# hdm0922/PathTracerDemo

Hardware: AMD Instinct MI355X
Metric: Msamples/sec at 1920x1080, 1 spp ReSTIR DI; per-pixel L2 vs WebGPU ref (higher is better)
Workload: dtype f32; 1 GPU; c3_interior_32 reuse 1920x1080, 1 spp/frame (configs[2]); frame=1920x1080, band_rows_per_gpu=1080, parallelism=row-bands x1

## Files before the change

pathtracerdemo_amd/csrc/ptx_api.cpp:

```cpp
#include <hip/hip_runtime.h>

#include <algorithm>
#include <cmath>
#include <cstdarg>
#include <cstdlib>
#include <cstdio>
#include <cstring>
#include <new>
#include <string>
#include <unordered_map>
#include <vector>

#include "ptx_internal.h"

namespace ptx {


[[maybe_unused]] static const char *const kShippedKnobs[] = {"COMM_TIMEOUT_S", "DEBUG_FILL", "HALO_PROXY_US"};
#if defined(PTX_WG_TIMES)
static const char *const kBuildKind = "wgt";
#elif defined(PTX_AB_BUILD)
static const char *const kBuildKind = "ab";
#else
static const char *const kBuildKind = "product";
// ... 351 lines not shown
    if (mats.size() != 8u * subs.size()) return fail(h, PTX_E_SCENE, "material / sub-mesh tables disagree");
    for (size_t k = 0; k < subs.size(); ++k) std::memcpy(&subs[k].pad, &mats[8u * k + 5u], 4);
    if (int rc = upload(h, h->d_tris, tris.data(), tris.size() * sizeof(float))) return rc;
    if (int rc = upload(h, h->d_nodes, nodes.data(), nodes.size() * sizeof(NodePair))) return rc;
    if (int rc = upload(h, h->d_subs, subs.data(), subs.size() * sizeof(SubRoot))) return rc;
    h->n_subs = (uint32_t)subs.size();
    if (int rc = upload(h, h->d_insts, insts.data(), std::max<size_t>(1, insts.size()) * sizeof(Inst))) return rc;
    if (int rc = upload(h, h->d_mats, mats.data(), mats.size() * sizeof(float))) return rc;
    if (int rc = upload(h, h->d_tverts, tverts.data(), tverts.size() * sizeof(float))) return rc;
    h->n_tris = (uint32_t)(tris.size() / 12);
    h->n_nodes = (uint32_t)nodes.size();
    h->n_inst = n_inst;
    h->max_depth = max_depth;
    h->stack_depth = max_depth + 2u;
    if ((size_t)h->stack_depth * kBlock * 4u > 160u * 1024u)
        return fail(h, PTX_E_SCENE, "BLAS depth %u needs more LDS than a CU has", max_depth);
    h->layout_valid = true;
    for (auto &c : h->ctx) c.surf_valid = false;
    gbuf_key_drop_all(h);
    return PTX_OK;
}

Scene make_scene(ptx_handle *h) {
    Scene sc{};
    std::memcpy(sc.U, h->uniform, sizeof sc.U);
    sc.S = (const uint32_t *)h->d_scene.p;
    sc.G = (const uint32_t *)h->d_geometry.p;
    sc.tris = (const float4 *)h->d_tris.p;
    sc.nodes = (const NodePair *)h->d_nodes.p;
    sc.subs = (const SubRoot *)h->d_subs.p;
    sc.insts = (const Inst *)h->d_insts.p;
    sc.mats = (const float4 *)h->d_mats.p;
    sc.tverts = (const float4 *)h->d_tverts.p;
    sc.n_inst = h->n_inst;
    sc.n_subs = h->n_subs;
    sc.width = h->cfg.width;
    sc.height = h->cfg.height;
    sc.row_begin = h->cfg.row_begin;
    sc.row_end = h->cfg.row_end;
    sc.counters = (h->cfg.flags & PTX_FLAG_COUNT_WORK) ? (unsigned long long *)h->d_counters.p : nullptr;
    sc.census = (h->cfg.flags & PTX_FLAG_ROW_CENSUS) ? (unsigned long long *)h->d_census.p : nullptr;
    sc.frame_color = (float4 *)h->d_frame_color.p;
#ifdef PTX_WG_TIMES
    sc.wgt = (unsigned long long *)h->d_wgt.p;
#endif
    return sc;
}

void resolve_event(TimedLaunch &t, ptx_handle *h) {
    if (!t.pending) return;
    float ms = 0.0f;
    if (hipEventSynchronize(t.stop) == hipSuccess && hipEventElapsedTime(&ms, t.start, t.stop) == hipSuccess) {
        h->ms_total[t.pass] += ms;
        h->launches[t.pass] += 1;
    }
    t.pending = false;
}

static uint32_t seg_pixels(const ptx_handle *h) {
    static const uint32_t env_px = (uint32_t)ab_knob("SEG_PX", 0);
    if (env_px >= 256u && env_px <= 8192u && env_px % 256u == 0u) return env_px;
    const size_t npx = (size_t)h->band_h * h->cfg.width;
    if ((h->cfg.pipeline == PTX_PIPELINE_RESTIR && restir_pipe()) || (h->cfg.pipeline == PTX_PIPELINE_MCPT && mcpt_pipe()) ||
        h->cfg.pipeline == PTX_PIPELINE_RESTIR_GI) {
        const size_t p = (npx / 1152u + 128u) / 256u * 256u;
        return (uint32_t)std::min<size_t>(4096u, std::max<size_t>(kWaveSegPixels, p));
// ... 1763 lines not shown
```

pathtracerdemo_amd/csrc/ptx_device.h:

```cpp
#pragma once

#include <hip/hip_runtime.h>
#include <stdint.h>

namespace ptx {

constexpr uint32_t STRIDE_INSTANCE = 33u;
constexpr uint32_t STRIDE_LIGHT = 18u;
constexpr uint32_t STRIDE_DESCRIPTOR = 6u;
constexpr uint32_t STRIDE_MATERIAL = 15u;
constexpr uint32_t STRIDE_VERTEX = 8u;
constexpr float RECONNECTION_DISTANCE = 0.1f;
constexpr float RECONNECTION_ROUGHNESS = 0.5f;
constexpr float INF_F = 1e11f;
constexpr float EPS_F = 1e-4f;
constexpr float PI_F = 3.141592f;
constexpr float ENV_C = 0.5f;
constexpr uint32_t LIGHT_DIRECTION = 0u, LIGHT_POINT = 1u, LIGHT_RECT = 2u, LIGHT_ENV = 3u;
constexpr uint32_t LOBE_LAMBERT = 0u, LOBE_GGX = 1u, LOBE_LIGHT = 3u;

enum : uint32_t {
    U_W = 0, U_H = 1, U_VPINV = 4, U_CAMPOS = 20, U_FRAME = 23, U_OFF_DESC = 24, U_OFF_MAT = 25,
    U_OFF_LIGHT = 26, U_OFF_CDF = 27, U_OFF_INDEX = 28, U_OFF_SUBROOT = 29, U_OFF_BLAS = 30,
    U_INST_COUNT = 31, U_LIGHT_COUNT = 32
};

constexpr uint32_t LEAF_BIT = 0x80000000u;
constexpr uint32_t LEAF_FIRST_MASK = 0x00FFFFFFu;

struct alignas(16) NodePair {
    float x[4], y[4], z[4];
    uint32_t lref, rref, pad0, pad1;
};
struct alignas(16) SubRoot {
    float x[2], y[2], z[2];
    uint32_t ref;
    uint32_t pad;
};
struct alignas(16) Inst {
    float m[16];
    float minv[16];
    uint32_t mesh, sub_base, nsub, tri_base;
    float wlo[3], wpad;
    float whi[3], wscale;
};
constexpr uint32_t kInstIdentity = 0x80000000u;

struct Scene {
    uint32_t U[33];
    const uint32_t *S;
    const uint32_t *G;
    const float4 *tris;
    const NodePair *nodes;
    const SubRoot *subs;
    const Inst *insts;
    const float4 *mats;
    const float4 *tverts;
    uint32_t n_inst, n_subs;
    uint32_t width, height, row_begin, row_end;
    unsigned long long *counters;
    unsigned long long *census;
    float4 *frame_color;
#ifdef PTX_WG_TIMES
    unsigned long long *wgt;
#endif
};

enum : uint32_t { KID_TRACE = 1, KID_GBUF, KID_INIT_START, KID_INIT_STEP, KID_FINAL_START, KID_FINAL_STEP,
                  KID_TEMP_START, KID_TEMP_COMBINE, KID_SPAT_START, KID_JOB_STEP, KID_SPAT_COMBINE };
#ifdef PTX_WG_TIMES
struct WaveTimer {
    unsigned long long *buf;
    unsigned long long t0;
    uint32_t kid;
    __device__ WaveTimer(unsigned long long *b, uint32_t k) : buf(b), t0(__builtin_amdgcn_s_memrealtime()), kid(k) {}
    __device__ ~WaveTimer() {
        if (!buf || __lane_id() != 0u) return;
        const unsigned long long t1 = __builtin_amdgcn_s_memrealtime();
        const unsigned long long i = atomicAdd(buf, 1ull);
        if (i >= (1ull << 20)) return;
        unsigned long long *r = buf + 4u + 4u * i;
        r[0] = t0;
        r[1] = t1;
        r[2] = ((unsigned long long)kid << 32) | blockIdx.x;
        r[3] = ((unsigned long long)(threadIdx.x >> 6) << 32) | (unsigned long long)__builtin_amdgcn_s_getreg((31 << 11) | 4);
    }
};
#define PTX_WAVE_TIMER(sc, k) WaveTimer wave_timer_((sc).wgt, (k))
constexpr uint32_t KID_BATCH = 12;
constexpr uint32_t KID_BATCH_DBG = 15;
// ... 725 lines not shown
    if ((COUNT || PROF) && counted) {
        atomicAdd(&sc.counters[CNT_RAYS], 1ull);
        atomicAdd(&sc.counters[CNT_INST], (unsigned long long)sc.n_inst);
        atomicAdd(&sc.counters[CNT_AABB], (unsigned long long)n_aabb);
        atomicAdd(&sc.counters[CNT_TRI], (unsigned long long)n_tri);
        if (best.valid) atomicAdd(&sc.counters[CNT_HITS], 1ull);
    }
    if (best.valid) {
        best.t = vy;
        if (!ANY && want_pos) complete_hit(sc, ray, eps, best, insts);
    }
    return best;
}

constexpr uint32_t kLdsTableMax = 24576u;
__host__ __device__ __forceinline__ uint32_t tables_lds_bytes(const Scene &sc) {
    return ((sc.n_subs * (uint32_t)sizeof(SubRoot) + 15u) & ~15u) + sc.n_inst * (uint32_t)sizeof(Inst);
}
__host__ __device__ __forceinline__ bool tables_fit_lds(const Scene &sc) { return tables_lds_bytes(sc) <= kLdsTableMax; }
struct LdsTables { const SubRoot *subs; const Inst *insts; };
__device__ __forceinline__ LdsTables stage_tables(const Scene &sc, uint32_t *lds) {
    SubRoot *l_subs = reinterpret_cast<SubRoot *>(lds);
    Inst *l_insts = reinterpret_cast<Inst *>(lds + ((sc.n_subs * (uint32_t)sizeof(SubRoot) + 15u) & ~15u) / 4u);
    const uint32_t *gs = reinterpret_cast<const uint32_t *>(sc.subs);
    uint32_t *ls = reinterpret_cast<uint32_t *>(l_subs);
    for (uint32_t i = threadIdx.x; i < sc.n_subs * (uint32_t)(sizeof(SubRoot) / 4u); i += blockDim.x) ls[i] = gs[i];
    const uint32_t *gi = reinterpret_cast<const uint32_t *>(sc.insts);
    uint32_t *li = reinterpret_cast<uint32_t *>(l_insts);
    for (uint32_t i = threadIdx.x; i < sc.n_inst * (uint32_t)(sizeof(Inst) / 4u); i += blockDim.x) li[i] = gi[i];
    __syncthreads();
    return LdsTables{l_subs, l_insts};
}

template <bool COUNT, bool PROF = false>
__device__ __forceinline__ Hit trace_core(const Scene &sc, Ray ray, PassEps eps, uint32_t *stack, uint32_t stride,
                                          float t_max = 1e10f) {
    return trace_core_tab<COUNT, PROF>(sc, sc.subs, sc.insts, ray, eps, stack, stride, t_max);
}
template <bool COUNT>
__device__ __attribute__((noinline)) Hit trace_ray(const Scene &sc, Ray ray, PassEps eps, uint32_t *stack,
                                                  uint32_t stride) {
    return trace_core<COUNT>(sc, ray, eps, stack, stride);
}

}
```

pathtracerdemo_amd/csrc/ptx_launch.h:

```cpp
#pragma once

#include <hip/hip_runtime.h>

#include "ptx_device.h"

namespace ptx {

constexpr int kTile = 16;
constexpr int kBlock = 256;

int env_knob(const char *key, int dflt);
#ifdef PTX_AB_BUILD
inline int ab_knob(const char *key, int dflt) { return env_knob(key, dflt); }
#else
constexpr int ab_knob(const char *, int dflt) { return dflt; }
#endif

inline size_t stack_lds_bytes(uint32_t depth) { return (size_t)depth * kBlock * sizeof(uint32_t); }

hipError_t launch_gbuffer(const Scene &sc, uint4 *gbuf, uint32_t stack_depth, hipStream_t s);
hipError_t launch_init(const Scene &sc, const uint4 *gbuf, uint4 *reservoir, uint32_t stack_depth, hipStream_t s);
hipError_t launch_final(const Scene &sc, const uint4 *gbuf, const uint4 *reservoir, float4 *accum,
                        uint32_t stack_depth, hipStream_t s);
hipError_t launch_mcpt(const Scene &sc, float4 *accum, uint32_t stack_depth, hipStream_t s);
hipError_t launch_present(const float4 *tex, uint32_t W, uint32_t H, uint32_t cw, uint32_t ch, bool bgra,
                          uint32_t *out, hipStream_t s);

struct DnWin {
    uint32_t y0;
    uint32_t rows;
    uint32_t c0, c1;
};
struct DnImage {
    const float4 *own, *halo;
    uint32_t o0, o1;
};
hipError_t launch_denoise_guide(const Scene &sc, const uint4 *gbuf, float4 *guide, float sigma_plane, hipStream_t s);
hipError_t launch_denoise_guide_halo(const Scene &sc, const uint4 *texels, uint32_t top, uint32_t bottom, float4 *guide,
                                     float sigma_plane, hipStream_t s);
hipError_t launch_denoise_variance(uint32_t W, const DnWin &win, const DnImage &img, const float4 *guide, float4 *out,
                                   hipStream_t s);
hipError_t launch_denoise_atrous(uint32_t W, const DnWin &win, uint32_t step, const float4 *in, const float4 *guide,
                                 float4 *out, float sigma_lum, bool last, hipStream_t s);
hipError_t launch_denoise_temporal(uint32_t W, uint32_t H, const DnWin &win, const float *vp_prev, float alpha_min,
                                   uint32_t mode, uint32_t prev_y0, uint32_t prev_rows, const float4 *guide,
                                   const float4 *frame, const float4 *accum, const float4 *pguide, const float4 *phist,
                                   const float2 *pmom, float4 *hist, float2 *mom, unsigned long long *clip, hipStream_t s);
hipError_t launch_denoise_variance_moments(uint32_t W, const DnWin &win, const float4 *hist, const float2 *mom,
                                           const float4 *guide, float4 *out, hipStream_t s);
// ... 119 lines not shown
```

pathtracerdemo_amd/csrc/ptx_reuse.hip:

```cpp
#include "ptx_wave_common.h"

namespace ptx {

constexpr uint32_t SALT_TEMPORAL = 0x54454D50u, SALT_SPATIAL = 0x53504154u;

enum : uint32_t { JS_HDR, JS_F, JS_CUR, JS_NRM, JS_PREV, JS_RRF, JS_COUNT };
constexpr uint32_t kJobFresh = 1u << 24;
constexpr uint32_t kResReuseLayout = 0x100u;
#ifndef PTX_JOB_FRESH
#define PTX_JOB_FRESH 1
#endif

struct Job {
    uint32_t i, length, phase, seed1, idx, matref;
    uint32_t k, lab;
    bool shift, rok;
    int32_t ref;
    int32_t dom;
    f3 f;
    float prod;
    Surface cur;
    f3 prev;
    float beta, rr_p;
    f3 rr_f;
// ... 198 lines not shown
                const f3 Ld = normalize(r);
                gl = fabsf(dot(get_light(sc, (uint32_t)XL.id).dir, Ld)) / dot(r, r);
            }
            s.prod = hyb ? s.prod / s.beta : s.prod / (gl * s.beta);
            Le = l_emit<true>(XL, s.cur);
            s.phase = 1u;
            const float dist = length(XL.pos - s.cur.pos);
            o = s.cur.pos; d = (XL.pos - s.cur.pos) / dist; remain = dist;
            vis = true;
            ray = go = ok;
        }
        if (!go) A.jres[jid] = make_float4(0.0f, 0.0f, 0.0f, 0.0f);
    }
    const uint32_t idx = g.rbase + wave_alloc(g.l_ray, ray ? 1u : 0u);
    if (ray) {
        s.idx = idx;
        put_ray(g.rays, idx, o, d, remain, vis ? Q_VIS : Q_CLOSEST);
        if (vis) g.res_out[2u * idx] = make_float4(0.0f, Le.x, Le.y, Le.z);
    }
    return go;
}

__device__ __forceinline__ void job_finish(const Seg &g, const JobLists &JL, const ReuseArgs &A, bool live,
                                           const Job &s, uint32_t jid) {
    if (live) job_store(A, jid, s);
    const bool fold = live && A.fold_last && s.phase == 1u;
    if (fold) A.jres[jid] = make_float4(asf(s.idx), asf(g.out_sel), 0.0f, asf(kJobPending));
    job_keep(g, JL, live && !fold, live && s.phase == 1u, jid);
}

#ifndef JOB_STEP_WAVES
#define JOB_STEP_WAVES 4
#endif
__device__ __forceinline__ uint32_t job_step_segment(const Scene &sc, const WaveBufs &w, uint32_t round,
                                                     const ReuseArgs &A, uint32_t *lds) {
    const JobLists JL = job_lists(w, lds);
    const Seg g = seg_begin(w, round, lds);
    uint32_t nh;
    const uint32_t n = split_count(g, nh);
    for (uint32_t base = 0; base < n; base += WB) {
        const uint32_t q = base + threadIdx.x;
        bool emit = false;
        uint32_t jid = 0u;
        Job s;
        if (q < n) {
            jid = split_at(g, JL, q, nh);
            job_load(sc, A, jid, s);
            if (s.phase != 1u) {
                bool ok = true;
                Surface next;
                uint32_t nref = 0u;
                if (s.phase == 0u) {
                    const Hit h = get_hit(g.res_in, s.idx);
                    ok = h.valid;
                    if (ok) {
                        next = surface_at(sc, h.s, h.pos);
                        nref = mat_index(sc, h.s.inst, h.s.mat);
                    }
                } else {
                    const uint4 *rv = res_of(A, s.ref);
                    const Compact cc = gdecode(s.phase == 2u ? rv[4] : rc_next(rv, rv[5].x));
                    next = get_surface(sc, cc);
                    nref = mat_index(sc, cc.inst, cc.mat);
                    if (s.phase == 2u) {
                        const Hit h = get_hit(g.res_in, s.idx);
                        ok = !(h.valid && h.t < length(next.pos - s.cur.pos) * 0.999f);
                    }
                }
                if (!ok) {
                    A.jres[jid] = make_float4(0.0f, 0.0f, 0.0f, 0.0f);
                } else {
                    const f3 V = normalize(s.prev - s.cur.pos);
                    const f3 L = normalize(next.pos - s.cur.pos);
                    s.f = s.f * (bsdf(s.cur, L, V) * fabsf(dot(s.cur.nrm, L)));
                    if (s.phase == 2u || (!s.shift && job_hyb(s) && s.i + 1u == s.k))
                        s.prod = s.prod * rc_geo(s.cur.pos, next);
                    s.prev = s.cur.pos;
                    s.cur = next;
                    s.matref = nref;
                    s.i += 1u;
                    emit = true;
                }
            } else {
                const float4 a = g.res_in[2u * s.idx];
                s.f = s.f * (mk(a.y, a.z, a.w) * a.x);
                const float qv = s.prod;
                const bool valid = qv > 0.0f && qv <= 3.402823466e38f;
                A.jres[jid] = valid ? make_float4(s.f.x, s.f.y, s.f.z, qv) : make_float4(0.0f, 0.0f, 0.0f, 0.0f);
            }
        }
        const bool live = job_emit(sc, g, A, emit, s, jid, 0u);
        job_finish(g, JL, A, live, s, jid);
    }
    job_seg_end(w, g, JL);
    return *g.l_ray;
}
__global__ __launch_bounds__(WB) __attribute__((amdgpu_waves_per_eu(JOB_STEP_WAVES, 8)))
void wjob_step(Scene sc, WaveBufs w, uint32_t round, ReuseArgs A) {
    PTX_WAVE_TIMER(sc, KID_JOB_STEP | (w.seg_base ? 0x80u : 0u));
    __shared__ uint32_t lds[3];
    (void)job_step_segment(sc, w, round, A, lds);
}

__device__ __forceinline__ uint32_t reuse_seed(const Scene &sc, uint32_t x, uint32_t y, uint32_t salt) {
    return pcg(pcg(x * 1973u + y * 9277u + sc.U[U_FRAME] * 26699u) ^ salt);
}
__device__ __forceinline__ bool wrs_update(float &w_sum, float wt, uint32_t &seed) {
    w_sum += wt;
    return rnd(seed) < wt / w_sum;
}
struct SelF { bool known; f3 f; };
__device__ __forceinline__ SelF job_f(float4 r) { return SelF{r.w > 0.0f, mk(r.x, r.y, r.z)}; }
__device__ __forceinline__ float4 job_result(const ReuseArgs &A, const WaveBufs &w, float4 r, uint32_t jid) {
    if (asu(r.w) != kJobPending || asu(r.x) >= A.ray_cap || asu(r.y) >= w.nres) return r;
    const float4 a = w.res[asu(r.y)][2u * asu(r.x)], fv = A.jstate[JS_F * (size_t)A.njobs + jid];
    const f3 f = mk(fv.x, fv.y, fv.z) * (mk(a.y, a.z, a.w) * a.x);
    const float qv = fv.w;
    const bool valid = qv > 0.0f && qv <= 3.402823466e38f;
    return valid ? make_float4(f.x, f.y, f.z, qv) : make_float4(0.0f, 0.0f, 0.0f, 0.0f);
}
__device__ __forceinline__ float4 job_at(const ReuseArgs &A, const WaveBufs &w, uint32_t pix, uint32_t slot) {
    const uint32_t jid = job_id(A, pix, slot);
    return job_result(A, w, A.jres[jid], jid);
}
__device__ __forceinline__ SelF stored_f(const uint4 *r) {
    const uint4 r6 = r[6], r7 = r[7];
    return SelF{r7.w == 1u, mk(asf(r6.z), asf(r6.w), asf(r7.z))};
}
__device__ __forceinline__ uint32_t write_reused(uint4 *out, const uint4 *src, float p_sel, float q_sel, SelF fs,
                                                 float w_sum, uint32_t C) {
    uint4 a0 = src[0], a5 = src[5];
    const uint4 a1 = src[1], a2 = src[2], a3 = src[3], a4 = src[4];
    if (fs.known && !(a5.x & kResReuseLayout)) {
        const uint32_t k = a5.x & 0xffu;
// ... 31 lines not shown
            return false;
        }
        const float4 c = w.state[(s.i == 1u ? kStateCs2 : kStateCs3) * w.npix + pix];
        const Surface next = get_surface(sc, gdecode(make_uint4(asu(c.x), asu(c.y), asu(c.z), asu(c.w))));
        V = normalize(s.prev - s.cur.pos);
        const f3 L = normalize(next.pos - s.cur.pos);
        s.f = s.f * (bsdf(s.cur, L, V) * fabsf(dot(s.cur.nrm, L)));
        if (hyb && s.i + 1u == s.k) s.prod = s.prod * rc_geo(s.cur.pos, next);
        s.prev = s.cur.pos;
        s.cur = next;
        s.i += 1u;
    }
    const float T = w.state[kStateTsel * w.npix + pix].x;
    if (T < 0.0f) return true;
    const LightSample XL = load_xl(rv);
    const f3 V = normalize(s.prev - s.cur.pos);
    const f3 L = direction_to_light(s.cur, XL);
    s.f = s.f * (bsdf(s.cur, L, V) * fabsf(dot(s.cur.nrm, L)));
    float gl = 1.0f;
    if (XL.type == LIGHT_RECT) {
        const f3 r = XL.pos - s.cur.pos;
        const f3 Ld = normalize(r);
        gl = fabsf(dot(get_light(sc, (uint32_t)XL.id).dir, Ld)) / dot(r, r);
    }
    s.prod = hyb ? s.prod / s.beta : s.prod / (gl * s.beta);
    const f3 Le = l_emit<true>(XL, s.cur);
    s.f = s.f * (Le * T);
    const float qv = s.prod;
    const bool valid = qv > 0.0f && qv <= 3.402823466e38f;
    A.jres[jid] = valid ? make_float4(s.f.x, s.f.y, s.f.z, qv) : make_float4(0.0f, 0.0f, 0.0f, 0.0f);
    return false;
}

__global__ __launch_bounds__(WB) __attribute__((amdgpu_waves_per_eu(2, 8)))
void wtemporal_start(Scene sc, WaveBufs w, ReuseArgs A) {
    PTX_WAVE_TIMER(sc, KID_TEMP_START | (w.seg_base ? 0x80u : 0u));
    __shared__ uint32_t lds[3];
    const JobLists JL = job_lists(w, lds);
    const Seg g = seg_begin(w, 0u, lds);
    const uint32_t np = padded_pixels(sc);
    for (uint32_t k = 0; k < w.seg_px; k += WB) {
        const uint32_t q = seg_pixel(w, g.j, k);
        uint32_t x, y, pix = 0u;
        bool active = false;
        Job s;
        if (q < np && tile_xy(sc, q, x, y)) {
            pix = (y - sc.row_begin) * sc.width + x;
            active = job_begin(sc, A, s, x, y, (int32_t)pix, (int32_t)pix);
            if (active && A.use_init) active = temporal_from_init(sc, w, A, s, pix, pix);
        }
        const bool live = job_emit(sc, g, A, active, s, pix, active ? A.cur[8u * (size_t)pix].x : 0u);
        job_finish(g, JL, A, live, s, pix);
    }
    job_seg_end(w, g, JL);
}

__global__ __launch_bounds__(WB) void wtemporal_combine(Scene sc, WaveBufs w, ReuseArgs A) {
    PTX_WAVE_TIMER(sc, KID_TEMP_COMBINE | (w.seg_base ? 0x80u : 0u));
    const uint32_t j = w.seg_base + blockIdx.x, np = padded_pixels(sc);
    for (uint32_t k = 0; k < w.seg_px; k += WB) {
        const uint32_t q = seg_pixel(w, j, k);
        uint32_t x, y;
        if (q >= np || !tile_xy(sc, q, x, y)) continue;
        const uint32_t pix = (y - sc.row_begin) * sc.width + x;
        if (!gdecode(A.gbuf[pix]).valid) {
            A.nbr_out[pix] = make_uint4(0u, 0u, 0u, 0u);
            continue;
        }
        uint4 *rv = A.cur + 8u * (size_t)pix;
        const uint4 *hv = A.hist + 8u * (size_t)pix;
        uint32_t seed = reuse_seed(sc, x, y, SALT_TEMPORAL);
// ... 32 lines not shown
    const float *vp = A.vp_prev;
    const f3 P = X1.pos;
    const float cx = ((vp[0] * P.x + vp[4] * P.y) + vp[8] * P.z) + vp[12];
    const float cy = ((vp[1] * P.x + vp[5] * P.y) + vp[9] * P.z) + vp[13];
    const float cw = ((vp[3] * P.x + vp[7] * P.y) + vp[11] * P.z) + vp[15];
    if (!(cw > 0.0f)) return m;
    const float W = (float)sc.width, H = (float)sc.height;
    const float fx = ((cx / cw + 1.0f) * 0.5f) * W, fy = ((cy / cw + 1.0f) * 0.5f) * H;
    if (!(fx >= 0.0f && fx < W && fy >= 0.0f && fy < H)) return m;
    m.px = (uint32_t)fx;
    m.py = (uint32_t)fy;
    const int32_t ry = (int32_t)m.py - (int32_t)sc.row_begin;
    if (abs((int32_t)m.py - (int32_t)y) > (int32_t)A.radius || ry < A.prev_row_lo || ry >= A.prev_row_hi) {
        if (count && A.clip) atomicAdd(A.clip, 1ull);
        return m;
    }
    m.pp = ry * (int32_t)sc.width + (int32_t)m.px;
    const uint4 a = A.psurf[2 * (ptrdiff_t)m.pp];
    if (a.w == kNoSurface) return m;
    const uint4 b = A.psurf[2 * (ptrdiff_t)m.pp + 1];
    const f3 pp = mk(asf(a.x), asf(a.y), asf(a.z)), pn = mk(asf(b.x), asf(b.y), asf(b.z));
    if (!(dot(pn, X1.nrm) >= 0.9f)) return m;
    const f3 x0p = x0_prev(A, sc, m.px, m.py);
    const float dp = length(pp - x0p), dc = length(P - x0p);
    if (!(fabsf(dp - dc) <= 0.05f * dc)) return m;
    m.C = min(A.hist[8 * (ptrdiff_t)m.pp + 7].y, A.cap);
    m.ok = m.C != 0u;
    return m;
}

#ifndef MOTION_START_WAVES
#define MOTION_START_WAVES 3
#endif
__global__ __launch_bounds__(WB) __attribute__((amdgpu_waves_per_eu(MOTION_START_WAVES, 8)))
void wtmotion_start(Scene sc, WaveBufs w, ReuseArgs A) {
    PTX_WAVE_TIMER(sc, KID_TEMP_START | (w.seg_base ? 0x80u : 0u));
    __shared__ uint32_t lds[3];
    const JobLists JL = job_lists(w, lds);
    const Seg g = seg_begin(w, 0u, lds);
    const uint32_t np = padded_pixels(sc);
    for (uint32_t k = 0; k < w.seg_px; k += WB) {
        const uint32_t q = seg_pixel(w, g.j, k);
        uint32_t x = 0u, y = 0u, pix = 0u;
        bool valid = false;
        Surface X1{};
        uint32_t mref = 0u;
        if (q < np && tile_xy(sc, q, x, y)) {
            pix = (y - sc.row_begin) * sc.width + x;
            valid = surf_load(sc, A.surf, pix, X1, mref);
        }
        const uint4 *rv = A.cur + 8u * (size_t)pix;
        const uint4 r5c = valid ? rv[5] : make_uint4(0u, 0u, 0u, 0u);
        const uint32_t cC = valid ? rv[7].y : 0u, clen = r5c.w, ck = r5c.x & 0xffu;
        const bool canon = valid && cC != 0u && clen >= 2u;
        const MotionHist mh = valid ? motion_hist(sc, A, X1, y, true) : MotionHist{false, 0, 0u, 0u, 0u};
#pragma unroll 1
        for (uint32_t slot = 0; slot < kMotionJobs; ++slot) {
            const uint32_t jid = job_id(A, pix, slot);
            Job s;
            bool act = false;
            uint32_t s0 = 0u;
            if (slot == 0u) {
                act = canon && job_begin(sc, A, s, x, y, (int32_t)pix, (int32_t)pix);
                if (act && A.use_init) act = temporal_from_init(sc, w, A, s, pix, jid);
                if (act) s0 = rv[0].x;
            } else if (slot == 1u) {
                if (mh.ok) {
                    const uint4 *hv = A.hist + 8 * (ptrdiff_t)mh.pp;
                    const uint4 h0 = hv[0], h5 = hv[5], h6 = hv[6];
                    act = h5.w >= 2u && asf(h6.x) > 0.0f;
                    if (act) {
// ... 535 lines not shown
__global__ __launch_bounds__(WB) void wspatial_combine(Scene sc, WaveBufs w, ReuseArgs A) {
    PTX_WAVE_TIMER(sc, KID_SPAT_COMBINE | (w.seg_base ? 0x80u : 0u));
    const uint32_t j = w.seg_base + blockIdx.x, np = padded_pixels(sc);
    for (uint32_t k = 0; k < w.seg_px; k += WB) {
        const uint32_t q = seg_pixel(w, j, k);
        uint32_t x, y, pix = 0u;
        bool replay = false;
        if (q < np && tile_xy(sc, q, x, y)) {
            pix = (y - sc.row_begin) * sc.width + x;
            if (!gdecode(A.gbuf[pix]).valid) {
                uint4 *out = A.hist + 8u * (size_t)pix;
                for (int t = 0; t < 8; ++t) out[t] = make_uint4(0u, 0u, 0u, 0u);
                if (A.fuse_final)
                    (void)shade_reused(sc, A, mix_weight(sc), A.accum[pix], pix, false, 0u, 0u,
                                       SelF{false, mk(0.0f, 0.0f, 0.0f)}, 0.0f);
            } else if (A.neighbors == 3u) {
                replay = combine_pixel<3>(sc, A, w, x, y, pix);
            } else {
                replay = combine_pixel<0>(sc, A, w, x, y, pix);
            }
        }
        if (A.fuse_final) replay_append(A, w, w.seg_phys + j, replay, pix);
    }
}

int reuse_rounds(int pass_temporal, const ReuseArgs &A) {
    return pass_temporal && A.use_init && !A.motion ? 1 : kWaveRoundsReuse;
}

hipError_t wave_reuse_round(const Scene &sc, const WaveBufs &w, int pass_temporal, int round, const ReuseArgs &A,
                            hipStream_t s) {
    const dim3 grid(w.seg_count), blk(WB);
    if (round == 0) {
        if (pass_temporal && A.motion) hipLaunchKernelGGL(wtmotion_start, grid, blk, 0, s, sc, w, A);
        else if (pass_temporal) hipLaunchKernelGGL(wtemporal_start, grid, blk, 0, s, sc, w, A);
        else hipLaunchKernelGGL(wspatial_start, grid, blk, 0, s, sc, w, A);
    } else if (round <= reuse_rounds(pass_temporal, A)) {
        hipLaunchKernelGGL(wjob_step, grid, blk, 0, s, sc, w, (uint32_t)round, A);
    } else {
        if (pass_temporal && A.motion) hipLaunchKernelGGL(wtmotion_combine, grid, blk, 0, s, sc, w, A);
        else if (pass_temporal) hipLaunchKernelGGL(wtemporal_combine, grid, blk, 0, s, sc, w, A);
        else if (A.neighbors == 3u && !ab_knob("COMBINE_SCALAR", 0))
            hipLaunchKernelGGL(wspatial_combine_shfl, dim3(w.seg_count), blk, 0, s, sc, w, A);
        else hipLaunchKernelGGL(wspatial_combine, grid, blk, 0, s, sc, w, A);
    }
    return hipGetLastError();
}

}
```

pathtracerdemo_amd/csrc/ptx_shading.h:

```cpp
#pragma once

#include "ptx_device.h"

namespace ptx {

struct Material { f3 albedo; float metal, rough, trans, ior; };
struct Surface { f3 pos, nrm; Material mat; };

__device__ __forceinline__ uint32_t mat_index(const Scene &sc, uint32_t inst, uint32_t sub) {
    return sc.insts[inst].sub_base + sub;
}
__device__ __forceinline__ Material material_at(const Scene &sc, uint32_t flat) {
    const float4 a = sc.mats[2u * flat], b = sc.mats[2u * flat + 1u];
    Material m;
    m.albedo = mk(a.x, a.y, a.z);
    m.metal = a.w;
    m.rough = b.x;
    m.trans = b.y;
    m.ior = b.z;
    return m;
}
__device__ __forceinline__ float get_transmission(const Scene &sc, uint32_t inst, uint32_t mid) {
    return sc.mats[2u * mat_index(sc, inst, mid) + 1u].y;
}
// ... 14 lines not shown
    f3 n2 = inst_point_t(I, I.minv, tv.n[2]);
    float U = x.bu, V = x.bv, W = 1.0f - U - V;
    s.nrm = normalize((n0 * U + n1 * V) + n2 * W);
    s.pos = (p0 * U + p1 * V) + p2 * W;
    return s;
}
__device__ __forceinline__ Surface surface_at(const Scene &sc, const Compact &x, f3 pos) {
    const Inst &I = sc.insts[x.inst];
    Surface s;
    s.mat = material_at(sc, I.sub_base + x.mat);
    const TriVerts tv = tri_verts(sc, I.tri_base + x.prim);
    f3 n0 = inst_point_t(I, I.minv, tv.n[0]);
    f3 n1 = inst_point_t(I, I.minv, tv.n[1]);
    f3 n2 = inst_point_t(I, I.minv, tv.n[2]);
    float U = x.bu, V = x.bv, W = 1.0f - U - V;
    s.nrm = normalize((n0 * U + n1 * V) + n2 * W);
    s.pos = pos;
    return s;
}
__device__ __forceinline__ f3 get_surface_pos(const Scene &sc, Compact x) {
    const Inst &I = sc.insts[x.inst];
    const TriVerts tv = tri_verts(sc, I.tri_base + x.prim);
    f3 p0 = inst_point(I, I.m, tv.p[0]);
    f3 p1 = inst_point(I, I.m, tv.p[1]);
    f3 p2 = inst_point(I, I.m, tv.p[2]);
    float U = x.bu, V = x.bv, W = 1.0f - U - V;
    return (p0 * U + p1 * V) + p2 * W;
}

struct Light { f3 pos, dir, color, U, V; uint32_t type; float intensity, area; };
struct LightSample { f3 dir; uint32_t type; f3 pos; int32_t id; f3 Le; float pdf; };

__device__ __forceinline__ Light get_light(const Scene &sc, uint32_t id) {
    const uint32_t *p = sc.S + sc.U[U_OFF_LIGHT] + STRIDE_LIGHT * id;
    Light l;
    l.pos = mk(asf(p[0]), asf(p[1]), asf(p[2]));
    l.dir = mk(asf(p[3]), asf(p[4]), asf(p[5]));
    l.color = mk(asf(p[6]), asf(p[7]), asf(p[8]));
    l.U = mk(asf(p[9]), asf(p[10]), asf(p[11]));
    l.V = mk(asf(p[12]), asf(p[13]), asf(p[14]));
    l.type = p[15];
    l.intensity = asf(p[16]);
    l.area = asf(p[17]);
    return l;
}
__device__ __forceinline__ float light_cdf(const Scene &sc, uint32_t i) { return asf(sc.S[sc.U[U_OFF_CDF] + i]); }

__device__ __forceinline__ float ggx_d(float NdotH, float R) {
    float a = R * R, a2 = a * a;
    float X = NdotH * NdotH * (a2 - 1.0f) + 1.0f;
    float denom = PI_F * X * X;
    return a2 / fmaxf(denom, EPS_F);
}
__device__ __forceinline__ float geom_shadow(float NdotV, float NdotL, float R) {
    float r = R + 1.0f;
    float K = r * r / 8.0f;
    return 1.0f / ((NdotV * (1.0f - K) + K) * (NdotL * (1.0f - K) + K));
}
__device__ __forceinline__ float pow5(float x) {
    float x2 = x * x;
    return (x2 * x2) * x;
}
__device__ __forceinline__ void fsincos(float x, float &s, float &c) {
    int j = (int)(x * 1.27323954473516f);
    float y = (float)j;
    if (j & 1) {
        j += 1;
        y += 1.0f;
    }
    j &= 7;
    float z = ((x - y * 0.78515625f) - y * 2.4187564849853515625e-4f) - y * 3.77489497744594108e-8f;
    float zz = z * z;
    float ps = ((-1.9515295891e-4f * zz + 8.3321608736e-3f) * zz - 1.6666654611e-1f) * zz * z + z;
    float pc = ((2.443315711809948e-5f * zz - 1.388731625493765e-3f) * zz + 4.166664568298827e-2f) * zz * zz -
               0.5f * zz + 1.0f;
    const bool swap = (j & 2) != 0;
    const float sv = swap ? pc : ps, cv = swap ? ps : pc;
    s = (j == 4 || j == 6) ? -sv : sv;
    c = (j == 2 || j == 4) ? -cv : cv;
// ... 274 lines not shown
```

pathtracerdemo_amd/csrc/ptx_wave.hip:

```cpp
#include "ptx_wave_common.h"

#include <algorithm>
#include <cstdlib>

namespace ptx {

#ifndef TRACE_OCC_WAVES
#define TRACE_OCC_WAVES 5
#endif
#ifndef TRACE_COOP
#define TRACE_COOP true
#endif
#ifndef PTX_NODE_UNI
#define PTX_NODE_UNI 1
#endif
#ifndef PTX_FLAT_INST
#define PTX_FLAT_INST 1
#endif
constexpr uint32_t kFlatMinInstances = 1u;
#ifndef PTX_LDS_TRANS
#define PTX_LDS_TRANS 1
#endif
template <bool COUNT, bool PROF, bool OCC, bool LDS_TABLES, bool FLAT>
__device__ __forceinline__ void trace_lanes(const Scene &sc, const SubRoot *subs, const Inst *insts, PassEps eps,
// ... 481 lines not shown
        s.bsdf_idx = bbase;
        put_ray(rays, bbase, s.xpos, s.L, -1.0f, Q_CLOSEST);
    }
}

__device__ __forceinline__ void winit_store(float4 *state, uint32_t npix, uint32_t pix, const WInit &s) {
    state[IS_HDR * npix + pix] = make_float4(asf(s.seed), asf(s.i | (s.flags << 8)), asf(s.C), asf(s.vis_idx));
    state[IS_FP * npix + pix] = make_float4(s.f.x, s.f.y, s.f.z, s.p);
    state[IS_RES * npix + pix] = make_float4(s.w_sum, s.p_hat_sel, s.pdf_env, asf(s.bsdf_idx));
    state[IS_X * npix + pix] = make_float4(s.xpos.x, s.xpos.y, s.xpos.z, s.xrough);
    state[IS_XL * npix + pix] = make_float4(s.xlpos.x, s.xlpos.y, s.xlpos.z, asf(s.nee_seed));
    state[IS_L * npix + pix] = make_float4(s.L.x, s.L.y, s.L.z, 0.0f);
    state[IS_BSEED * npix + pix] = make_float4(asf(s.bseed1), asf(s.bseed2), 0.0f, 0.0f);
}
__device__ __forceinline__ void winit_load(const float4 *state, uint32_t npix, uint32_t pix, WInit &s) {
    const float4 h = state[IS_HDR * npix + pix], fp = state[IS_FP * npix + pix], r = state[IS_RES * npix + pix];
    const float4 x = state[IS_X * npix + pix], xl = state[IS_XL * npix + pix], l = state[IS_L * npix + pix];
    const float4 b = state[IS_BSEED * npix + pix];
    s.seed = asu(h.x); s.i = asu(h.y) & 0xffu; s.flags = asu(h.y) >> 8; s.C = asu(h.z); s.vis_idx = asu(h.w);
    s.f = mk(fp.x, fp.y, fp.z); s.p = fp.w;
    s.w_sum = r.x; s.p_hat_sel = r.y; s.pdf_env = r.z; s.bsdf_idx = asu(r.w);
    s.xpos = mk(x.x, x.y, x.z); s.xrough = x.w;
    s.xlpos = mk(xl.x, xl.y, xl.z); s.nee_seed = asu(xl.w);
    s.L = mk(l.x, l.y, l.z);
    s.bseed1 = asu(b.x); s.bseed2 = asu(b.y);
}
__device__ __forceinline__ void winit_finish(const WInit &s, uint4 *reservoir, uint32_t pix) {
    uint4 *out = reservoir + 8u * (size_t)pix;
    if (!(s.flags & F_SEL))
        for (int q = 0; q < 7; ++q) out[q] = make_uint4(0u, 0u, 0u, 0u);
    out[7] = make_uint4(asu(s.w_sum / s.p_hat_sel), s.C, 0u, 0u);
}

__global__ __launch_bounds__(WB) __attribute__((amdgpu_waves_per_eu(LOGIC_WAVES, 8))) void winit_start(Scene sc, WaveBufs w, const uint4 *gbuf, uint4 *reservoir) {
    PTX_WAVE_TIMER(sc, KID_INIT_START | (w.seg_base ? 0x80u : 0u));
    __shared__ uint32_t lds[3];
    const JobLists JL = job_lists(w, lds);
    const Seg g = seg_begin(w, 0u, lds);
    float4 *state = w.state;
    const uint32_t npix = w.npix, np = padded_pixels(sc);
    for (uint32_t k = 0; k < w.seg_px; k += WB) {
        const uint32_t q = seg_pixel(w, g.j, k);
        uint32_t x, y, pix = 0u;
        bool active = false;
        WInit s;
        Surface X;
        f3 prev;
        if (q < np && tile_xy(sc, q, x, y)) {
            pix = (y - sc.row_begin) * sc.width + x;
            const Compact x1 = gdecode(gbuf[pix]);
            if (!x1.valid) {
                uint4 *out = reservoir + 8u * (size_t)pix;
                for (int q8 = 0; q8 < 8; ++q8) out[q8] = make_uint4(0u, 0u, 0u, 0u);
                if (w.surf) surf_store_none(w.surf, pix);
            } else {
                active = true;
                s.seed = pcg(x * 1973u + y * 9277u + sc.U[U_FRAME] * 26699u);
                s.i = 1u; s.flags = 0u; s.C = 0u;
                s.f = mk(1.0f, 1.0f, 1.0f); s.p = 1.0f;
                s.w_sum = 0.0f; s.p_hat_sel = 0.0f; s.pdf_env = 0.0f;
                s.L = mk(0.0f, 0.0f, 0.0f); s.bseed1 = 0u; s.bseed2 = 0u; s.bsdf_idx = 0u;
                prev = x0_of(sc, x, y);
                X = get_surface(sc, x1);
                if (w.surf) surf_store(w.surf, pix, X, mat_index(sc, x1.inst, x1.mat));
                if (X.mat.rough >= RECONNECTION_ROUGHNESS) s.flags |= F_R1;
            }
        }
        winit_vertex(sc, g, active, s, X, prev);
        if (active) winit_store(state, npix, pix, s);
        job_keep(g, JL, active, active && !(s.flags & F_BSDF), pix);
    }
    job_seg_end(w, g, JL);
}

__global__ __launch_bounds__(WB) __attribute__((amdgpu_waves_per_eu(LOGIC_WAVES, 8))) void winit_step(Scene sc, WaveBufs w, uint32_t round, uint4 *reservoir) {
    PTX_WAVE_TIMER(sc, KID_INIT_STEP | (w.seg_base ? 0x80u : 0u));
    __shared__ uint32_t lds[3];
    const JobLists JL = job_lists(w, lds);
    const Seg g = seg_begin(w, round, lds);
    float4 *state = w.state;
    const float4 *res_in = g.res_in;
    const uint32_t npix = w.npix;
    uint32_t nh;
    const uint32_t n = split_count(g, nh);
    for (uint32_t base = 0; base < n; base += WB) {
        const uint32_t q = base + threadIdx.x;
        bool emit = false;
        uint32_t pix = 0u;
        WInit s;
        Surface X;
        f3 prev;
        if (q < n) {
            pix = split_at(g, JL, q, nh);
            winit_load(state, npix, pix, s);
            const float4 a = res_in[2u * s.vis_idx], b = res_in[2u * s.vis_idx + 1u];
            const f3 contrib = mk(a.y, a.z, a.w) * a.x;
            const float p_hat = luminance(contrib);
            const float ris = p_hat / b.x;
            s.C += 1u;
            s.w_sum += ris;
            if (b.y < ris / s.w_sum) {
                s.flags |= F_SEL;
                s.p_hat_sel = p_hat;
                state[IS_TSEL * npix + pix] = make_float4(a.x, 0.0f, 0.0f, 0.0f);
                LightSample XL;
                const Light ls = get_light(sc, asu(b.w));
                XL.id = (int32_t)asu(b.w);
                XL.type = ls.type;
                XL.Le = ls.color * ls.intensity;
                XL.pos = s.xlpos;
                XL.pdf = b.z;
// ... 566 lines not shown
}

hipError_t launch_trace_rays_sm(const Scene &sc, const float4 *rays, float4 *hits, uint32_t n, int eps_mode,
                                uint32_t depth, hipStream_t s) {
    if (n == 0) return hipSuccess;
    const PassEps eps = eps_mode == 0 ? PassEps{1e-8f, 1e-6f} : PassEps{1e-4f, 1e-8f};
    const uint32_t per_wg = 4u * WB;
    const dim3 grid((n + per_wg - 1u) / per_wg);
    if (sc.counters)
        hipLaunchKernelGGL(trace_queue_sm<true>, grid, dim3(WB), stack_lds_bytes(depth), s, sc, rays, hits, nullptr,
                           per_wg, n, eps);
    else
        hipLaunchKernelGGL(trace_queue_sm<false>, grid, dim3(WB), stack_lds_bytes(depth), s, sc, rays, hits, nullptr,
                           per_wg, n, eps);
    return hipGetLastError();
}

hipError_t wave_gbuffer(const Scene &sc, const WaveBufs &w, uint4 *gbuf, uint32_t depth, hipStream_t s) {
    if (!tables_fit_lds(sc)) return hipErrorInvalidValue;
    static const bool rootq = ab_knob("GBUF_ROOTQ", 0) != 0;
    if (rootq)
        hipLaunchKernelGGL(wgbuffer<true>, dim3(w.seg_px / WB * w.seg_count), dim3(WB),
                           tables_lds_bytes(sc) + stack_lds_bytes(depth), s, sc,
                           w, gbuf);
    else
        hipLaunchKernelGGL(wgbuffer<false>, dim3(w.seg_px / WB * w.seg_count), dim3(WB),
                           tables_lds_bytes(sc) + stack_lds_bytes(depth), s,
                           sc, w, gbuf);
    return hipGetLastError();
}

hipError_t wave_init_round(const Scene &sc, const WaveBufs &w, int round, const uint4 *gbuf, uint4 *reservoir,
                           hipStream_t s) {
    if (round == 0)
        hipLaunchKernelGGL(winit_start, dim3(w.seg_count), dim3(WB), 0, s, sc, w, gbuf, reservoir);
    else
        hipLaunchKernelGGL(winit_step, dim3(w.seg_count), dim3(WB), 0, s, sc, w, (uint32_t)round, reservoir);
    return hipGetLastError();
}

hipError_t wave_final_round(const Scene &sc, const WaveBufs &w, int round, const uint4 *gbuf, const uint4 *reservoir,
                            float4 *accum, hipStream_t s) {
    if (round == 0)
        hipLaunchKernelGGL(wfinal_start, dim3(w.seg_count), dim3(WB), 0, s, sc, w, gbuf, reservoir, accum);
    else
        hipLaunchKernelGGL(wfinal_step, dim3(w.seg_count), dim3(WB), 0, s, sc, w, (uint32_t)round, reservoir, accum);
    return hipGetLastError();
}

hipError_t wave_final_one(const Scene &sc, const WaveBufs &w, const uint4 *gbuf, const uint4 *reservoir, float4 *accum,
                          uint32_t depth, hipStream_t s) {
    const PassEps eps{1e-4f, 1e-8f};
    const size_t lds = tables_lds_bytes(sc) + stack_lds_bytes(depth);
    static const uint32_t flat_min = (uint32_t)ab_knob("FLAT_MIN_INST", (int)kFlatMinInstances);
    if (PTX_FLAT_INST && sc.n_inst >= flat_min)
        hipLaunchKernelGGL(wfinal_one<true>, dim3(w.seg_count), dim3(WB), lds, s, sc, w, gbuf, reservoir, accum, eps);
    else
        hipLaunchKernelGGL(wfinal_one<false>, dim3(w.seg_count), dim3(WB), lds, s, sc, w, gbuf, reservoir, accum, eps);
    return hipGetLastError();
}

hipError_t wave_final_replay(const Scene &sc, const WaveBufs &w, const uint4 *gbuf, const uint4 *reservoir, float4 *accum,
                             const uint32_t *replay, uint32_t *replay_cnt, uint32_t depth, hipStream_t s) {
    const PassEps eps{1e-4f, 1e-8f};
    const size_t lds = tables_lds_bytes(sc) + stack_lds_bytes(depth);
    static const uint32_t flat_min = (uint32_t)ab_knob("FLAT_MIN_INST", (int)kFlatMinInstances);
    if (PTX_FLAT_INST && sc.n_inst >= flat_min)
        hipLaunchKernelGGL(wfinal_replay<true>, dim3(w.seg_count), dim3(WB), lds, s, sc, w, gbuf, reservoir, accum, replay,
                           replay_cnt, eps);
    else
// ... 31 lines not shown
```

pathtracerdemo_amd/csrc/ptx_wave_common.h:

```cpp
#pragma once
#include "ptx_launch.h"
#include "ptx_shading.h"

namespace ptx {

constexpr uint32_t WB = kBlock;
#ifndef LOGIC_WAVES
#define LOGIC_WAVES 4
#endif
enum : uint32_t { Q_CLOSEST = 0u, Q_VIS = 1u, Q_OCC = 2u };

__device__ __forceinline__ uint32_t wave_scan(uint32_t v, uint32_t &total) { return wave_excl_sum(v, total); }
__device__ __forceinline__ uint32_t wave_alloc(uint32_t *lds_ctr, uint32_t n) {
    uint32_t total;
    const uint32_t excl = wave_scan(n, total);
    uint32_t base = 0u;
    if (__lane_id() == 0u && total) base = atomicAdd(lds_ctr, total);
    base = (uint32_t)__builtin_amdgcn_readfirstlane((int)base);
    return base + excl;
}

struct Seg {
    uint32_t j, round;
    uint32_t pj;
    uint32_t rbase;
    float4 *rays, *res_out;
    const float4 *res_in;
    uint32_t out_sel;
    uint32_t *act_out;
    const uint32_t *act_in;
    uint32_t n_in;
    uint32_t *l_ray, *l_act;
};
__device__ __forceinline__ uint32_t res_sel(const WaveBufs &w, uint32_t round) {
    return w.nres == 3u ? round % 3u : round & 1u;
}
__device__ __forceinline__ float4 *res_buf(const WaveBufs &w, uint32_t round) { return w.res[res_sel(w, round)]; }
__device__ __forceinline__ Seg seg_begin(const WaveBufs &w, uint32_t round, uint32_t *lds) {
    Seg g;
    g.j = w.seg_base + blockIdx.x;
    g.pj = w.seg_phys + g.j;
    g.round = round;
    g.rbase = g.pj * w.ray_stride;
    g.rays = w.rays;
    g.res_out = res_buf(w, round);
    g.res_in = round ? res_buf(w, round - 1u) : w.res[1];
    g.out_sel = res_sel(w, round);
    g.act_out = w.act[round & 1u] + (size_t)g.pj * w.act_stride;
    g.act_in = w.act[(round + 1u) & 1u] + (size_t)g.pj * w.act_stride;
    g.n_in = round ? w.cnt[(2u * (round - 1u)) * w.cnt_stride + g.pj] : 0u;
    g.l_ray = lds;
    g.l_act = lds + 1;
    if (threadIdx.x == 0) { lds[0] = 0u; lds[1] = 0u; }
    if (w.dyn && blockIdx.x == 0 && threadIdx.x < kDynHeads) w.dyn[round * kDynRoundWords + threadIdx.x * kDynStride] = 0u;
    __syncthreads();
    return g;
}
__device__ __forceinline__ void seg_end(const WaveBufs &w, const Seg &g) {
    __syncthreads();
    if (threadIdx.x == 0) {
        w.cnt[(2u * g.round) * w.cnt_stride + g.pj] = *g.l_act;
        w.cnt[(2u * g.round + 1u) * w.cnt_stride + g.pj] = *g.l_ray;
    }
}
__device__ __forceinline__ uint32_t set_tile(const WaveBufs &w, uint32_t v) {
    return v < w.ntile0 ? w.tile0 + v : v - w.ntile0 < w.ntile1 ? w.tile1 + (v - w.ntile0) : 0x3ffffffu;
}
__device__ __forceinline__ uint32_t seg_pixel(const WaveBufs &w, uint32_t j, uint32_t k) {
    const uint32_t s = (k + threadIdx.x) >> 6;
    const uint32_t cl = w.cluster;
    const uint32_t t = set_tile(w, ((s / cl) * w.nseg + j) * cl + s % cl);
    return t * 64u + (threadIdx.x & 63u);
}
__device__ __forceinline__ void seg_keep(const Seg &g, bool keep, uint32_t pix) {
    const uint32_t slot = wave_alloc(g.l_act, keep ? 1u : 0u);
    if (keep) g.act_out[slot] = pix;
}

struct JobLists { uint32_t *l_light; uint32_t stride; };
__device__ __forceinline__ JobLists job_lists(const WaveBufs &w, uint32_t *lds) {
    if (threadIdx.x == 0) lds[2] = 0u;
    return JobLists{lds + 2, w.act_stride};
}
// ... 103 lines not shown
```

Measured before the change: 584.2 Msamples/s.

## Stage instances, materials, lights and light CDF into LDS for shading kernels

```diff
diff --git a/pathtracerdemo_amd/csrc/ptx_api.cpp b/pathtracerdemo_amd/csrc/ptx_api.cpp
--- a/pathtracerdemo_amd/csrc/ptx_api.cpp
+++ b/pathtracerdemo_amd/csrc/ptx_api.cpp
@@ -407,6 +407,8 @@
     sc.insts = (const Inst *)h->d_insts.p;
     sc.mats = (const float4 *)h->d_mats.p;
     sc.tverts = (const float4 *)h->d_tverts.p;
+    sc.lights = sc.S ? sc.S + sc.U[U_OFF_LIGHT] : nullptr;
+    sc.cdf = sc.S ? sc.S + sc.U[U_OFF_CDF] : nullptr;
     sc.n_inst = h->n_inst;
     sc.n_subs = h->n_subs;
     sc.width = h->cfg.width;
diff --git a/pathtracerdemo_amd/csrc/ptx_device.h b/pathtracerdemo_amd/csrc/ptx_device.h
--- a/pathtracerdemo_amd/csrc/ptx_device.h
+++ b/pathtracerdemo_amd/csrc/ptx_device.h
@@ -56,6 +56,8 @@
     const Inst *insts;
     const float4 *mats;
     const float4 *tverts;
+    const uint32_t *lights;
+    const uint32_t *cdf;
     uint32_t n_inst, n_subs;
     uint32_t width, height, row_begin, row_end;
     unsigned long long *counters;
@@ -847,6 +849,44 @@
     return LdsTables{l_subs, l_insts};
 }
 
+constexpr uint32_t kShadeLdsMax = 16384u;
+__host__ __device__ __forceinline__ uint32_t shade_sec(unsigned long long bytes) {
+    return bytes > 0x7fffffffull ? 0x7fffffffu : ((uint32_t)bytes + 15u) & ~15u;
+}
+__host__ __device__ __forceinline__ uint32_t shading_lds_bytes(const Scene &sc) {
+    const unsigned long long nl = sc.U[U_LIGHT_COUNT];
+    const unsigned long long b = (unsigned long long)shade_sec(sc.n_inst * (unsigned long long)sizeof(Inst)) +
+                                 shade_sec(sc.n_subs * 2ull * sizeof(float4)) + shade_sec(nl * STRIDE_LIGHT * 4ull) +
+                                 shade_sec(nl * 4ull);
+    return b > 0x7fffffffull ? 0x7fffffffu : (uint32_t)b;
+}
+__host__ __device__ __forceinline__ bool shading_fits_lds(const Scene &sc) { return shading_lds_bytes(sc) <= kShadeLdsMax; }
+__device__ __forceinline__ Scene stage_shading(const Scene &sc, uint32_t *lds, bool copy) {
+    const uint32_t nl = sc.U[U_LIGHT_COUNT];
+    const uint32_t n_i = sc.n_inst * (uint32_t)(sizeof(Inst) / 16u), n_m = sc.n_subs * 2u;
+    const uint32_t n_l = nl * STRIDE_LIGHT, n_c = nl;
+    uint4 *l_insts = reinterpret_cast<uint4 *>(lds), *l_mats = l_insts + n_i;
+    uint32_t *l_lights = reinterpret_cast<uint32_t *>(l_mats + n_m), *l_cdf = l_lights + ((n_l + 3u) & ~3u);
+    if (copy) {
+        const uint4 *gi = reinterpret_cast<const uint4 *>(sc.insts), *gm = reinterpret_cast<const uint4 *>(sc.mats);
+        for (uint32_t i = threadIdx.x; i < n_i; i += blockDim.x) l_insts[i] = gi[i];
+        for (uint32_t i = threadIdx.x; i < n_m; i += blockDim.x) l_mats[i] = gm[i];
+        for (uint32_t i = threadIdx.x; i < n_l; i += blockDim.x) l_lights[i] = sc.lights[i];
+        for (uint32_t i = threadIdx.x; i < n_c; i += blockDim.x) l_cdf[i] = sc.cdf[i];
+    }
+    Scene t = sc;
+    t.insts = reinterpret_cast<const Inst *>(l_insts);
+    t.mats = reinterpret_cast<const float4 *>(l_mats);
+    t.lights = l_lights;
+    t.cdf = l_cdf;
+    return t;
+}
+template <bool LDS_SHADE>
+__device__ __forceinline__ Scene shading_scene(const Scene &sc, uint32_t *lds, bool copy) {
+    if constexpr (LDS_SHADE) return stage_shading(sc, lds, copy);
+    else return sc;
+}
+
 template <bool COUNT, bool PROF = false>
 __device__ __forceinline__ Hit trace_core(const Scene &sc, Ray ray, PassEps eps, uint32_t *stack, uint32_t stride,
                                           float t_max = 1e10f) {
diff --git a/pathtracerdemo_amd/csrc/ptx_launch.h b/pathtracerdemo_amd/csrc/ptx_launch.h
--- a/pathtracerdemo_amd/csrc/ptx_launch.h
+++ b/pathtracerdemo_amd/csrc/ptx_launch.h
@@ -15,6 +15,13 @@
 #else
 constexpr int ab_knob(const char *, int dflt) { return dflt; }
 #endif
+
+enum : int { SL_INIT_START = 1, SL_INIT_STEP = 2, SL_TEMPORAL_START = 4, SL_JOB_STEP = 16 };
+inline bool shade_from_lds(const Scene &sc, int kernel_bit) {
+    static const int mask = ab_knob("SHADE_LDS", SL_INIT_START | SL_INIT_STEP | SL_TEMPORAL_START | SL_JOB_STEP);
+    return shading_fits_lds(sc) && (mask & kernel_bit) != 0;
+}
+inline size_t shade_lds_bytes(bool staged, const Scene &sc) { return staged ? shading_lds_bytes(sc) : 0u; }
 
 inline size_t stack_lds_bytes(uint32_t depth) { return (size_t)depth * kBlock * sizeof(uint32_t); }
 
diff --git a/pathtracerdemo_amd/csrc/ptx_reuse.hip b/pathtracerdemo_amd/csrc/ptx_reuse.hip
--- a/pathtracerdemo_amd/csrc/ptx_reuse.hip
+++ b/pathtracerdemo_amd/csrc/ptx_reuse.hip
@@ -254,9 +254,11 @@
 #ifndef JOB_STEP_WAVES
 #define JOB_STEP_WAVES 4
 #endif
-__device__ __forceinline__ uint32_t job_step_segment(const Scene &sc, const WaveBufs &w, uint32_t round,
-                                                     const ReuseArgs &A, uint32_t *lds) {
+template <bool LDS_SHADE>
+__device__ __forceinline__ uint32_t job_step_segment(const Scene &gsc, const WaveBufs &w, uint32_t round,
+                                                     const ReuseArgs &A, uint32_t *lds, uint32_t *shade_lds) {
     const JobLists JL = job_lists(w, lds);
+    const Scene sc = shading_scene<LDS_SHADE>(gsc, shade_lds, seg_n_in(w, round) != 0u);
     const Seg g = seg_begin(w, round, lds);
     uint32_t nh;
     const uint32_t n = split_count(g, nh);
@@ -317,11 +319,13 @@
     job_seg_end(w, g, JL);
     return *g.l_ray;
 }
+template <bool LDS_SHADE>
 __global__ __launch_bounds__(WB) __attribute__((amdgpu_waves_per_eu(JOB_STEP_WAVES, 8)))
 void wjob_step(Scene sc, WaveBufs w, uint32_t round, ReuseArgs A) {
     PTX_WAVE_TIMER(sc, KID_JOB_STEP | (w.seg_base ? 0x80u : 0u));
     __shared__ uint32_t lds[3];
-    (void)job_step_segment(sc, w, round, A, lds);
+    extern __shared__ __attribute__((aligned(16))) uint32_t shade_lds[];
+    (void)job_step_segment<LDS_SHADE>(sc, w, round, A, lds, shade_lds);
 }
 
 __device__ __forceinline__ uint32_t reuse_seed(const Scene &sc, uint32_t x, uint32_t y, uint32_t salt) {
@@ -419,11 +423,14 @@
     return false;
 }
 
+template <bool LDS_SHADE>
 __global__ __launch_bounds__(WB) __attribute__((amdgpu_waves_per_eu(2, 8)))
-void wtemporal_start(Scene sc, WaveBufs w, ReuseArgs A) {
-    PTX_WAVE_TIMER(sc, KID_TEMP_START | (w.seg_base ? 0x80u : 0u));
+void wtemporal_start(Scene gsc, WaveBufs w, ReuseArgs A) {
+    PTX_WAVE_TIMER(gsc, KID_TEMP_START | (w.seg_base ? 0x80u : 0u));
     __shared__ uint32_t lds[3];
+    extern __shared__ __attribute__((aligned(16))) uint32_t shade_lds[];
     const JobLists JL = job_lists(w, lds);
+    const Scene sc = shading_scene<LDS_SHADE>(gsc, shade_lds, true);
     const Seg g = seg_begin(w, 0u, lds);
     const uint32_t np = padded_pixels(sc);
     for (uint32_t k = 0; k < w.seg_px; k += WB) {
@@ -522,11 +529,14 @@
 #ifndef MOTION_START_WAVES
 #define MOTION_START_WAVES 3
 #endif
+template <bool LDS_SHADE>
 __global__ __launch_bounds__(WB) __attribute__((amdgpu_waves_per_eu(MOTION_START_WAVES, 8)))
-void wtmotion_start(Scene sc, WaveBufs w, ReuseArgs A) {
-    PTX_WAVE_TIMER(sc, KID_TEMP_START | (w.seg_base ? 0x80u : 0u));
+void wtmotion_start(Scene gsc, WaveBufs w, ReuseArgs A) {
+    PTX_WAVE_TIMER(gsc, KID_TEMP_START | (w.seg_base ? 0x80u : 0u));
     __shared__ uint32_t lds[3];
+    extern __shared__ __attribute__((aligned(16))) uint32_t shade_lds[];
     const JobLists JL = job_lists(w, lds);
+    const Scene sc = shading_scene<LDS_SHADE>(gsc, shade_lds, true);
     const Seg g = seg_begin(w, 0u, lds);
     const uint32_t np = padded_pixels(sc);
     for (uint32_t k = 0; k < w.seg_px; k += WB) {
@@ -1128,11 +1138,18 @@
                             hipStream_t s) {
     const dim3 grid(w.seg_count), blk(WB);
     if (round == 0) {
-        if (pass_temporal && A.motion) hipLaunchKernelGGL(wtmotion_start, grid, blk, 0, s, sc, w, A);
-        else if (pass_temporal) hipLaunchKernelGGL(wtemporal_start, grid, blk, 0, s, sc, w, A);
-        else hipLaunchKernelGGL(wspatial_start, grid, blk, 0, s, sc, w, A);
+        if (pass_temporal) {
+            const bool staged = shade_from_lds(sc, SL_TEMPORAL_START);
+            auto k = A.motion ? (staged ? wtmotion_start<true> : wtmotion_start<false>)
+                              : (staged ? wtemporal_start<true> : wtemporal_start<false>);
+            hipLaunchKernelGGL(k, grid, blk, shade_lds_bytes(staged, sc), s, sc, w, A);
+        } else {
+            hipLaunchKernelGGL(wspatial_start, grid, blk, 0, s, sc, w, A);
+        }
     } else if (round <= reuse_rounds(pass_temporal, A)) {
-        hipLaunchKernelGGL(wjob_step, grid, blk, 0, s, sc, w, (uint32_t)round, A);
+        const bool staged = shade_from_lds(sc, SL_JOB_STEP);
+        auto k = staged ? wjob_step<true> : wjob_step<false>;
+        hipLaunchKernelGGL(k, grid, blk, shade_lds_bytes(staged, sc), s, sc, w, (uint32_t)round, A);
     } else {
         if (pass_temporal && A.motion) hipLaunchKernelGGL(wtmotion_combine, grid, blk, 0, s, sc, w, A);
         else if (pass_temporal) hipLaunchKernelGGL(wtemporal_combine, grid, blk, 0, s, sc, w, A);
diff --git a/pathtracerdemo_amd/csrc/ptx_shading.h b/pathtracerdemo_amd/csrc/ptx_shading.h
--- a/pathtracerdemo_amd/csrc/ptx_shading.h
+++ b/pathtracerdemo_amd/csrc/ptx_shading.h
@@ -70,7 +70,7 @@
 struct LightSample { f3 dir; uint32_t type; f3 pos; int32_t id; f3 Le; float pdf; };
 
 __device__ __forceinline__ Light get_light(const Scene &sc, uint32_t id) {
-    const uint32_t *p = sc.S + sc.U[U_OFF_LIGHT] + STRIDE_LIGHT * id;
+    const uint32_t *p = sc.lights + STRIDE_LIGHT * id;
     Light l;
     l.pos = mk(asf(p[0]), asf(p[1]), asf(p[2]));
     l.dir = mk(asf(p[3]), asf(p[4]), asf(p[5]));
@@ -82,7 +82,7 @@
     l.area = asf(p[17]);
     return l;
 }
-__device__ __forceinline__ float light_cdf(const Scene &sc, uint32_t i) { return asf(sc.S[sc.U[U_OFF_CDF] + i]); }
+__device__ __forceinline__ float light_cdf(const Scene &sc, uint32_t i) { return asf(sc.cdf[i]); }
 
 __device__ __forceinline__ float ggx_d(float NdotH, float R) {
     float a = R * R, a2 = a * a;
diff --git a/pathtracerdemo_amd/csrc/ptx_wave.hip b/pathtracerdemo_amd/csrc/ptx_wave.hip
--- a/pathtracerdemo_amd/csrc/ptx_wave.hip
+++ b/pathtracerdemo_amd/csrc/ptx_wave.hip
@@ -537,10 +537,13 @@
     out[7] = make_uint4(asu(s.w_sum / s.p_hat_sel), s.C, 0u, 0u);
 }
 
-__global__ __launch_bounds__(WB) __attribute__((amdgpu_waves_per_eu(LOGIC_WAVES, 8))) void winit_start(Scene sc, WaveBufs w, const uint4 *gbuf, uint4 *reservoir) {
-    PTX_WAVE_TIMER(sc, KID_INIT_START | (w.seg_base ? 0x80u : 0u));
+template <bool LDS_SHADE>
+__global__ __launch_bounds__(WB) __attribute__((amdgpu_waves_per_eu(LOGIC_WAVES, 8))) void winit_start(Scene gsc, WaveBufs w, const uint4 *gbuf, uint4 *reservoir) {
+    PTX_WAVE_TIMER(gsc, KID_INIT_START | (w.seg_base ? 0x80u : 0u));
     __shared__ uint32_t lds[3];
+    extern __shared__ __attribute__((aligned(16))) uint32_t shade_lds[];
     const JobLists JL = job_lists(w, lds);
+    const Scene sc = shading_scene<LDS_SHADE>(gsc, shade_lds, true);
     const Seg g = seg_begin(w, 0u, lds);
     float4 *state = w.state;
     const uint32_t npix = w.npix, np = padded_pixels(sc);
@@ -578,10 +581,13 @@
     job_seg_end(w, g, JL);
 }
 
-__global__ __launch_bounds__(WB) __attribute__((amdgpu_waves_per_eu(LOGIC_WAVES, 8))) void winit_step(Scene sc, WaveBufs w, uint32_t round, uint4 *reservoir) {
-    PTX_WAVE_TIMER(sc, KID_INIT_STEP | (w.seg_base ? 0x80u : 0u));
+template <bool LDS_SHADE>
+__global__ __launch_bounds__(WB) __attribute__((amdgpu_waves_per_eu(LOGIC_WAVES, 8))) void winit_step(Scene gsc, WaveBufs w, uint32_t round, uint4 *reservoir) {
+    PTX_WAVE_TIMER(gsc, KID_INIT_STEP | (w.seg_base ? 0x80u : 0u));
     __shared__ uint32_t lds[3];
+    extern __shared__ __attribute__((aligned(16))) uint32_t shade_lds[];
     const JobLists JL = job_lists(w, lds);
+    const Scene sc = shading_scene<LDS_SHADE>(gsc, shade_lds, seg_n_in(w, round) != 0u);
     const Seg g = seg_begin(w, round, lds);
     float4 *state = w.state;
     const float4 *res_in = g.res_in;
@@ -1214,10 +1220,15 @@
 
 hipError_t wave_init_round(const Scene &sc, const WaveBufs &w, int round, const uint4 *gbuf, uint4 *reservoir,
                            hipStream_t s) {
-    if (round == 0)
-        hipLaunchKernelGGL(winit_start, dim3(w.seg_count), dim3(WB), 0, s, sc, w, gbuf, reservoir);
-    else
-        hipLaunchKernelGGL(winit_step, dim3(w.seg_count), dim3(WB), 0, s, sc, w, (uint32_t)round, reservoir);
+    const bool staged = shade_from_lds(sc, round == 0 ? SL_INIT_START : SL_INIT_STEP);
+    const size_t lds = shade_lds_bytes(staged, sc);
+    if (round == 0) {
+        auto k = staged ? winit_start<true> : winit_start<false>;
+        hipLaunchKernelGGL(k, dim3(w.seg_count), dim3(WB), lds, s, sc, w, gbuf, reservoir);
+    } else {
+        auto k = staged ? winit_step<true> : winit_step<false>;
+        hipLaunchKernelGGL(k, dim3(w.seg_count), dim3(WB), lds, s, sc, w, (uint32_t)round, reservoir);
+    }
     return hipGetLastError();
 }
 
diff --git a/pathtracerdemo_amd/csrc/ptx_wave_common.h b/pathtracerdemo_amd/csrc/ptx_wave_common.h
--- a/pathtracerdemo_amd/csrc/ptx_wave_common.h
+++ b/pathtracerdemo_amd/csrc/ptx_wave_common.h
@@ -36,6 +36,9 @@
     return w.nres == 3u ? round % 3u : round & 1u;
 }
 __device__ __forceinline__ float4 *res_buf(const WaveBufs &w, uint32_t round) { return w.res[res_sel(w, round)]; }
+__device__ __forceinline__ uint32_t seg_n_in(const WaveBufs &w, uint32_t round) {
+    return round ? w.cnt[(2u * (round - 1u)) * w.cnt_stride + w.seg_phys + w.seg_base + blockIdx.x] : 0u;
+}
 __device__ __forceinline__ Seg seg_begin(const WaveBufs &w, uint32_t round, uint32_t *lds) {
     Seg g;
     g.j = w.seg_base + blockIdx.x;
@@ -48,7 +51,7 @@
     g.out_sel = res_sel(w, round);
     g.act_out = w.act[round & 1u] + (size_t)g.pj * w.act_stride;
     g.act_in = w.act[(round + 1u) & 1u] + (size_t)g.pj * w.act_stride;
-    g.n_in = round ? w.cnt[(2u * (round - 1u)) * w.cnt_stride + g.pj] : 0u;
+    g.n_in = seg_n_in(w, round);
     g.l_ray = lds;
     g.l_act = lds + 1;
     if (threadIdx.x == 0) { lds[0] = 0u; lds[1] = 0u; }
```

Result: faster. 596.3 Msamples/s, median of 6 (+2.1%).
